# AbnerVictor/OOD-GAN-inversion

Hardware: AMD Instinct MI355X
Metric: 1024² face inversions/sec (100 W+ steps) (higher is better)
Workload: dtype f16-split (hi+lo f16 operands, f32 accumulate): 3 MFMA/product in every forward conv (fp32-equivalent), 2 in the input-gradient convs (back-propagated gradient rounded to f16 before each contraction, weights keep hi+lo); dL/dW+ vs the float64 reference 1.4e-5..3.6e-5 ('f16s': 1.3e-5..2.6e-5, the ref

## Files before the change

### ood-gan-inversion_amd/csrc/common.hpp

```cpp
#pragma once
#include <hip/hip_runtime.h>
#include <cstdio>
#include <cstdarg>
#include <functional>
#include <utility>
#include "../../include/oodgan.h"

namespace oodgan {
struct PlanRec;
extern thread_local PlanRec* tl_plan_rec;
extern int g_null_launch;
void plan_append(std::function<void()>&& f);
template <class F>
inline void launch_rec(F&& f) {
    f();
    if (__builtin_expect(tl_plan_rec != nullptr, 0)) plan_append(std::function<void()>(std::forward<F>(f)));
}
}
#undef hipLaunchKernelGGL
#define hipLaunchKernelGGL(kernelName, numBlocks, numThreads, memPerBlock, streamId, ...)                                        \
    ::oodgan::launch_rec([=]() {                                                                                                 \
        if (!::oodgan::g_null_launch) (kernelName)<<<(numBlocks), (numThreads), (memPerBlock), (streamId)>>>(__VA_ARGS__);      \
    })

namespace oodgan {

void set_error(const char* fmt, ...);

enum { OODGAN_TUN_S1_BIG_MIN_ITEMS = 0, OODGAN_TUN_S2_BIG_MIN_ITEMS, OODGAN_TUN_T2_BIG_MIN_ITEMS, OODGAN_TUN_BLURT_STRIP, OODGAN_TUN_BLUR_STRIP, OODGAN_TUN_UPVB_WAVES, OODGAN_TUN_FEWOUT_QUAD, OODGAN_TUN_TINY_MID_MAX, OODGAN_TUN_STRIPX_WAVES, OODGAN_TUN_COUNT };
long tunable(int id);

enum { OODGAN_DC_STRIPX = 0, OODGAN_DC_STRIP, OODGAN_DC_S1BIG, OODGAN_DC_S1V2, OODGAN_DC_S1PP, OODGAN_DC_TINY, OODGAN_DC_T2BIG,
       OODGAN_DC_T2V2, OODGAN_DC_T2GEN, OODGAN_DC_S2BIG, OODGAN_DC_S2V2, OODGAN_DC_S2GEN, OODGAN_DC_UPVB,
       OODGAN_DC_S1BIG_YS, OODGAN_DC_S2BIG_FUSE, OODGAN_DC_S2BIG_DOTXS,
       OODGAN_DC_S1BIG_G2, OODGAN_DC_S2BIG_G2, OODGAN_DC_STRIPX_G2, OODGAN_DC_S2BIG_XH, OODGAN_DC_S1BIG_XH,
       OODGAN_DC_COMPOSITE_MSE,
       OODGAN_DC_SSIM, OODGAN_DC_COUNT };
void count_dispatch(int id);

bool bound_device_ok(const char* what);

inline int check_launch(const char* what) {
    hipError_t e = hipGetLastError();
    if (e != hipSuccess) {
        set_error("%s: %s", what, hipGetErrorString(e));
        return OODGAN_E_LAUNCH;
    }
    return OODGAN_OK;
}

#define OODGAN_REQUIRE(cond, ...)          \
    do {                                    \
        if (!(cond)) {                      \
            oodgan::set_error(__VA_ARGS__); \
            return OODGAN_E_ARG;            \
        }                                   \
    } while (0)

constexpr float kSqrt2 = 1.4142135623730951f;
constexpr float kInvPos = 1.f / kSqrt2, kInvNeg = 1.f / (0.2f * kSqrt2);
constexpr int kWave = 64;

inline hipStream_t as_stream(void* s) { return reinterpret_cast<hipStream_t>(s); }

inline int stream_grid(long work_items, int block) {
    long g = (work_items + block - 1) / block;
    if (g > 2048) g = 2048;
    if (g < 1) g = 1;
    return static_cast<int>(g);
}

__device__ __forceinline__ float wave_sum(float v) {
#pragma unroll
    for (int o = 32; o > 0; o >>= 1) v += __shfl_xor(v, o, 64);
    return v;
}

__device__ __forceinline__ float row_sum16(const float* __restrict__ p, int n, int l) {
    float v[4];
#pragma unroll
    for (int u = 0; u < 4; ++u) v[u] = p[min(l + 16 * u, n - 1)];
#pragma unroll
    for (int u = 0; u < 4; ++u) v[u] = l + 16 * u < n ? v[u] : 0.f;
    float r = (v[0] + v[1]) + (v[2] + v[3]);
    r += __shfl_xor(r, 8, 64);
    r += __shfl_xor(r, 4, 64);
    r += __shfl_xor(r, 2, 64);
    r += __shfl_xor(r, 1, 64);
    return r;
}

__device__ __forceinline__ float row_sum_wave(const float* __restrict__ p, int n, int lane) {
    float a0 = 0.f, a1 = 0.f, a2 = 0.f, a3 = 0.f;
    for (int i0 = lane; i0 < n; i0 += 512) {
        float v[8];
#pragma unroll
        for (int u = 0; u < 8; ++u) v[u] = p[min(i0 + 64 * u, n - 1)];
#pragma unroll
        for (int u = 0; u < 8; ++u) v[u] = i0 + 64 * u < n ? v[u] : 0.f;
        a0 += v[0] + v[4]; a1 += v[1] + v[5]; a2 += v[2] + v[6]; a3 += v[3] + v[7];
    }
    return wave_sum((a0 + a1) + (a2 + a3));
}

__device__ __forceinline__ float row_sum(const float* __restrict__ p, int n, int lane) {
    return n <= 64 ? row_sum16(p, n, lane & 15) : row_sum_wave(p, n, lane);
}

__device__ __forceinline__ float demod_dot(const float* __restrict__ sp, const float* __restrict__ wp, int Ci, int lane) {
    float a0 = 0.f, a1 = 0.f, a2 = 0.f, a3 = 0.f;
    for (int c0 = lane; c0 < Ci; c0 += 512) {
        float sv[8], wv[8];
#pragma unroll
        for (int u = 0; u < 8; ++u) {
            const int ci = min(c0 + 64 * u, Ci - 1);
            sv[u] = sp[ci];
            wv[u] = wp[ci];
        }
#pragma unroll
        for (int u = 0; u < 8; ++u) {
            const float pr = c0 + 64 * u < Ci ? sv[u] * sv[u] * wv[u] : 0.f;
            if ((u & 3) == 0) a0 += pr; else if ((u & 3) == 1) a1 += pr; else if ((u & 3) == 2) a2 += pr; else a3 += pr;
        }
    }
    return wave_sum((a0 + a1) + (a2 + a3));
}

#ifndef OODGAN_NT_STREAM
#define OODGAN_NT_STREAM 1
#endif
typedef float oodgan_f4v __attribute__((ext_vector_type(4)));
typedef float oodgan_f2v __attribute__((ext_vector_type(2)));
typedef unsigned oodgan_u4v __attribute__((ext_vector_type(4)));
__device__ __forceinline__ float4 ld4_stream(const float* p) {
#if OODGAN_NT_STREAM
    const oodgan_f4v v = __builtin_nontemporal_load(reinterpret_cast<const oodgan_f4v*>(p));
    return make_float4(v.x, v.y, v.z, v.w);
#else
    return *reinterpret_cast<const float4*>(p);
#endif
}
__device__ __forceinline__ float2 ld2_stream(const float* p) {
#if OODGAN_NT_STREAM
    const oodgan_f2v v = __builtin_nontemporal_load(reinterpret_cast<const oodgan_f2v*>(p));
    return make_float2(v.x, v.y);
#else
    return *reinterpret_cast<const float2*>(p);
#endif
}
__device__ __forceinline__ float ld1_stream(const float* p) {
#if OODGAN_NT_STREAM
    return __builtin_nontemporal_load(p);
#else
    return *p;
#endif
}
__device__ __forceinline__ void st4_stream(float* p, float4 v) {
#if OODGAN_NT_STREAM
    __builtin_nontemporal_store(oodgan_f4v{v.x, v.y, v.z, v.w}, reinterpret_cast<oodgan_f4v*>(p));
#else
    *reinterpret_cast<float4*>(p) = v;
#endif
}
template <typename T16>
__device__ __forceinline__ void st16_stream(void* p, const T16& v) {
    static_assert(sizeof(T16) == 16, "16-byte value");
#if OODGAN_NT_STREAM
    __builtin_nontemporal_store(__builtin_bit_cast(oodgan_u4v, v), reinterpret_cast<oodgan_u4v*>(p));
#else
    *reinterpret_cast<T16*>(p) = v;
#endif
}

template <int CTRL, int ROW_MASK>
__device__ __forceinline__ float dpp_take(float v) {
    return __builtin_bit_cast(float, __builtin_amdgcn_update_dpp(0, __builtin_bit_cast(int, v), CTRL, ROW_MASK, 0xF, false));
}
__device__ __forceinline__ float half_sum_dpp(float v) {
    v += dpp_take<0xB1, 0xF>(v);
    v += dpp_take<0x4E, 0xF>(v);
    v += dpp_take<0x141, 0xF>(v);
    v += dpp_take<0x140, 0xF>(v);
    v += dpp_take<0x142, 0xA>(v);
    return v;
}
constexpr int kHalfSumLane = 31;

__device__ __forceinline__ float block_sum_256(float v, float* red ) {
    v = wave_sum(v);
    const int lane = threadIdx.x & 63, wv = threadIdx.x >> 6;
    __syncthreads();
    if (lane == 0) red[wv] = v;
    __syncthreads();
    return red[0] + red[1] + red[2] + red[3];
}

}
```

### ood-gan-inversion_amd/csrc/conv_f16s_s2big.hip

```cpp
#include "conv_common.hpp"
#include "sform.hpp"
#include <cstdint>
#include <cstdlib>
#include <type_traits>

using namespace oodgan;

typedef _Float16 half8 __attribute__((ext_vector_type(8)));
typedef __attribute__((address_space(3))) void lds_void;

#ifdef OODGAN_CLOCK_STAMP
__device__ unsigned long long* g_s2big_stamp = nullptr;
__device__ long g_s2big_stamp_n = 0;
#define S2_STAMP(i) do { if (FUSE && (wave == 0 || wave == 7)) stv[i] = __builtin_amdgcn_s_memtime(); } while (0)
#else
#define S2_STAMP(i)
#endif

namespace {

constexpr int SB_ROWS = 9, SB_C = 33;
constexpr int SB_ROWSLOTS = 2 * SB_C * 4;
constexpr int SB_XSLOTS = SB_ROWS * SB_ROWSLOTS;
constexpr int SB_XPIECES = 40;
constexpr int SB_XBYTES = SB_XPIECES * 1024;

struct SPDims2 { int KC, Hq, Wq; long plane; };

__host__ __device__ inline SPDims2 sp_dims2(int C, int H, int W) {
    SPDims2 d;
    d.KC = (C + 15) / 16;
    d.Hq = (H + 7) / 8 * 8 + 2;
    d.Wq = (W + 31) / 32 * 32 + 2;
    d.plane = (long)d.Hq * d.Wq * 4;
    return d;
}

struct S2Big {
    oodgan_conv_args a;
    const uint4* xs;
    SPDims2 sp;
    const float* w_unscale;
    int Hout, Wout, tiles_x, tiles_y, mblocks, Mp;
    long out_plane;
    int ablate;
    oodgan_actbwd_fuse f;
    SDims yd;
};

template <int MH>
struct S2Cfg {
    static constexpr int RW = MH == 2 ? 2 : 1;
    static constexpr int NRG = 8 / RW;
    static constexpr int MBW = 64 * MH;
    static constexpr int TAPB = 4 * MBW * 16;
    static constexpr int PPT = TAPB / 1024;
    static constexpr int WA = 6 * PPT / 8, WB = (3 * PPT + 7) / 8;
    static constexpr int NA = 5 + WA, NB = 5 + WB;
    static constexpr int OFF_XA = 0, OFF_WA = SB_XBYTES, OFF_XB = OFF_WA + 6 * TAPB, OFF_WB = OFF_XB + SB_XBYTES;
    static constexpr int SMEM = OFF_WB + 3 * TAPB;
    static constexpr int OFF_CST = SMEM;
    static constexpr int SMEM_FUSE = SMEM + 8 * MBW * 4;
};

constexpr int vmcnt_imm(int n) { return ((n >> 4) & 3) << 14 | 0x0F70 | (n & 15); }

typedef _Float16 half2v __attribute__((ext_vector_type(2)));

template <bool DOT, int MH, bool FUSE = false, bool G2 = false>
__global__ __launch_bounds__(512) void conv_f16s_s2big_kernel(const S2Big p, const uint4* __restrict__ wpk16) {
    using C = S2Cfg<MH>;
    constexpr int RW = C::RW;
    extern __shared__ __attribute__((aligned(16))) unsigned char smem[];
    const oodgan_conv_args& a = p.a;
    const int tid = threadIdx.x, lane = tid & 63;
    const int wave = __builtin_amdgcn_readfirstlane(tid >> 6);
    const int l31 = lane & 31, half = lane >> 5;
    const int rg = wave % C::NRG, mh = wave / C::NRG;

#ifdef OODGAN_CLOCK_STAMP
    unsigned long long stv[8] = {0, 0, 0, 0, 0, 0, 0, 0};
#endif
    S2_STAMP(0);
    int w = xcd_remap(blockIdx.x, gridDim.x);
    const int mblk = w % p.mblocks;
    w /= p.mblocks;
    const int ntile = p.tiles_x * p.tiles_y;
    const int tile = w % ntile, b = w / ntile;
    const int ty = tile / p.tiles_x, tx = tile % p.tiles_x;
    const int r0 = ty * 8, c0 = tx * 32, m0 = mblk * C::MBW;
    const int H = p.Hout, W = p.Wout, M = a.M;

    const bool xh = G2 && a.x_hi_only == 2;
    unsigned offx[5];
    bool xok[5];
#pragma unroll
    for (int i = 0; i < 5; ++i) {
        int P = (wave + 8 * i) * 64 + lane;
        if (P >= SB_XSLOTS) P = SB_XSLOTS - 1;
        const int row = P / SB_ROWSLOTS, rem = P % SB_ROWSLOTS;
        const int px = rem / (SB_C * 4), q = rem % (SB_C * 4);
        const int c = q >> 2, s = ((q & 3) - ((c >> 2) & 3)) & 3;
        if (xh) {
            offx[i] = (unsigned)(((long)px * p.sp.plane + ((long)(r0 + row) * p.sp.Wq + (c0 + c)) * 2 + (s & 1)) * 16);
            xok[i] = s < 2;
        } else {
            offx[i] = (unsigned)(((long)px * p.sp.plane + ((long)(r0 + row) * p.sp.Wq + (c0 + c)) * 4 + s) * 16);
            xok[i] = true;
        }
    }
    const long plane_bytes = p.sp.plane * 16;
    const int grp = a.groups > 1 ? m0 / (M / a.groups) : 0;
    const unsigned char* xb = reinterpret_cast<const unsigned char*>(p.xs) + ((long)b * p.sp.KC + (long)grp * ((a.K + 15) / 16)) * 4 * plane_bytes;
    const unsigned char* wb = reinterpret_cast<const unsigned char*>(wpk16) + (long)m0 * 16;
    const unsigned lane16 = lane * 16;
    const long wchunk_bytes = (long)36 * p.Mp * 16;
    const long wrow_bytes = (long)p.Mp * 16;
    const int nchunk = (a.K + 15) / 16;
    const int nstage = 2 * nchunk;

    auto dma_piece = [&](int st, int j) {
        const int t = st >> 1, py = st & 1;
        if (j < 5) {
            unsigned char* dx_ = smem + (py ? C::OFF_XB : C::OFF_XA);
            const unsigned char* xsrc = xb + ((long)t * 4 + py * 2) * plane_bytes;
            if (!G2 || xok[j])
                __builtin_amdgcn_global_load_lds((const __attribute__((address_space(1))) void*)(xsrc + offx[j]),
                                                 (lds_void*)(dx_ + (wave + 8 * j) * 1024), 16, 0, 0);
            return;
        }
        const int i = j - 5;
        const int nw = py ? C::WB : C::WA, npieces = (py ? 3 : 6) * C::PPT;
        if (i >= nw) return;
        unsigned char* dw_ = smem + (py ? C::OFF_WB : C::OFF_WA);
        const unsigned char* wsrc = wb + (long)t * wchunk_bytes;
        int pw = wave + 8 * i;
        if (pw >= npieces) pw -= 8;
        const int sl = pw / C::PPT, q = pw % C::PPT;
        const int tap = py ? 3 + sl : (sl / 3) * 6 + sl % 3;
        const int row = (q * 64) / C::MBW, j0 = (q * 64) % C::MBW;
        const unsigned char* sb = wsrc + (long)(tap * 4 + row) * wrow_bytes + j0 * 16;
        __builtin_amdgcn_global_load_lds((const __attribute__((address_space(1))) void*)(sb + lane16), (lds_void*)(dw_ + pw * 1024), 16, 0, 0);
    };
    auto dma_stage = [&](int st) {
#pragma unroll
        for (int j = 0; j < C::NA; ++j) dma_piece(st, j);
    };

    f32x16 acc[2][RW];
#pragma unroll
    for (int mt = 0; mt < 2; ++mt)
#pragma unroll
        for (int nt = 0; nt < RW; ++nt)
#pragma unroll
            for (int r = 0; r < 16; ++r) acc[mt][nt][r] = 0.f;

    unsigned lrd[2][2];
#pragma unroll
    for (int dxs = 0; dxs < 2; ++dxs)
#pragma unroll
        for (int lo = 0; lo < 2; ++lo) {
            const int c = dxs + l31;
            lrd[dxs][lo] = c * 64 + (((half + 2 * lo + ((c >> 2) & 3)) & 3) << 4);
        }
    const unsigned lwf = (half * C::MBW + mh * 64 + l31) * 16;

    struct Frag { half8 ah[2], al[2], bh[RW], bl[RW]; };
    auto load_tap = [&](Frag& f, const unsigned char* lx, const unsigned char* lw, auto sl_c) {
        constexpr int sl = decltype(sl_c)::value;
        constexpr int arow = sl / 3, kx = sl % 3;
#pragma unroll
        for (int mt = 0; mt < 2; ++mt) {
            f.ah[mt] = *reinterpret_cast<const half8*>(lw + sl * C::TAPB + (0 * 2) * C::MBW * 16 + mt * 32 * 16);
            f.al[mt] = *reinterpret_cast<const half8*>(lw + sl * C::TAPB + (1 * 2) * C::MBW * 16 + mt * 32 * 16);
        }
#pragma unroll
        for (int nt = 0; nt < RW; ++nt) {
            const unsigned char* xr = lx + ((rg * RW + nt + arow) * 2 + (kx & 1)) * (SB_C * 64);
            f.bh[nt] = *reinterpret_cast<const half8*>(xr + lrd[kx >> 1][0]);
            if (!G2) f.bl[nt] = *reinterpret_cast<const half8*>(xr + lrd[kx >> 1][1]);
        }
    };
    auto mfma_tap = [&](const Frag& f) {
#pragma unroll
        for (int mt = 0; mt < 2; ++mt)
#pragma unroll
            for (int nt = 0; nt < RW; ++nt) acc[mt][nt] = __builtin_amdgcn_mfma_f32_32x32x16_f16(f.ah[mt], f.bh[nt], acc[mt][nt], 0, 0, 0);
        if (!G2) {
#pragma unroll
        for (int mt = 0; mt < 2; ++mt)
#pragma unroll
            for (int nt = 0; nt < RW; ++nt) acc[mt][nt] = __builtin_amdgcn_mfma_f32_32x32x16_f16(f.ah[mt], f.bl[nt], acc[mt][nt], 0, 0, 0);
        }
#pragma unroll
        for (int mt = 0; mt < 2; ++mt)
#pragma unroll
            for (int nt = 0; nt < RW; ++nt) acc[mt][nt] = __builtin_amdgcn_mfma_f32_32x32x16_f16(f.al[mt], f.bh[nt], acc[mt][nt], 0, 0, 0);
    };
#define S2B_IC(n) std::integral_constant<int, n>{}
#define S2B_SB() __builtin_amdgcn_sched_barrier(0)

    constexpr bool EARLY = FUSE && MH == 1;
    float eq0 = 0.f, eq1 = 0.f, eq2 = 0.f, enz = 0.f, edv[EARLY ? 2 : 1][16];
    bool eok = false;
    if constexpr (EARLY) {
        static_assert(!EARLY || RW == 1, "one row per wave");
        const oodgan_actbwd_fuse& f = p.f;
        const int px = c0 + l31, py_ = r0 + rg;
        const long HW = (long)H * W, pix = (long)py_ * W + px;
        eok = py_ < H && px < W;
        if (eok) {
            if (f.g_rgb) {
                const float* gr = f.g_rgb + (long)b * 3 * HW + pix;
                eq0 = gr[0]; eq1 = gr[HW]; eq2 = gr[2 * HW];
            }
            if (f.noise) enz = (f.noise_w ? f.noise_w[0] : 1.f) * f.noise[(long)(f.noise_batch > 1 ? b : 0) * HW + pix];
        }
        if (a.dotx_sform) {
#pragma unroll
            for (int mt = 0; mt < 2; ++mt)
#pragma unroll
                for (int blk = 0; blk < 2; ++blk) {
                    const int kc = min((m0 + mh * 64 + mt * 32) / 16 + blk, p.yd.KC - 1);
                    const unsigned char* rec = reinterpret_cast<const unsigned char*>(a.dotx) +
                        sform_unit(p.yd, b, kc, min(py_, H - 1), min(px, W - 1), 0) * 16 + 8 * half;
#pragma unroll
                    for (int sl = 0; sl < 4; ++sl) {
                        const float2 t = *reinterpret_cast<const float2*>(rec + 16 * sl);
                        edv[EARLY ? mt : 0][8 * blk + 2 * sl] = t.x;
                        edv[EARLY ? mt : 0][8 * blk + 2 * sl + 1] = t.y;
                    }
                }
        } else {
#pragma unroll
            for (int mt = 0; mt < 2; ++mt) {
                const float* dr = a.dotx + ((long)b * M + m0 + mh * 64 + mt * 32) * HW + pix;
#pragma unroll
                for (int r = 0; r < 16; ++r) {
                    const int ch = (r & 3) + 8 * (r >> 2) + 4 * half;
                    edv[EARLY ? mt : 0][r] = (eok && m0 + mh * 64 + mt * 32 + ch < M) ? dr[(long)ch * HW] : 0.f;
                }
            }
        }
    }

    float cv[8] = {0.f, 0.f, 0.f, 0.f, 0.f, 0.f, 0.f, 1.f};
    if constexpr (FUSE) {
        const oodgan_actbwd_fuse& f = p.f;
        if (tid < C::MBW) {
            const int m = min(m0 + tid, M - 1);
            cv[0] = a.out_scale ? a.out_scale[(long)b * a.out_scale_stride + m] : 1.f;
            if (f.g_rgb) {
                cv[1] = f.w_rgb[0 * M + m];
                cv[2] = f.w_rgb[1 * M + m];
                cv[3] = f.w_rgb[2 * M + m];
                cv[4] = f.s_rgb[(long)b * f.s_rgb_stride + m];
            }
            if (f.bias) cv[5] = f.bias[m];
            cv[6] = f.dscale[(long)b * f.dscale_stride + m];
            if (a.dotx_sform) {
                const float sc = a.dotx_scale[(long)b * a.dotx_scale_stride + m];
                cv[7] = sc != 0.f ? 1.f / sc : 0.f;
            }
        }
    }
    dma_stage(0);
    if constexpr (FUSE) {
        if (tid < C::MBW) {
            const oodgan_actbwd_fuse& f = p.f;
            float* cst = reinterpret_cast<float*>(smem + C::OFF_CST);
            const bool mok = m0 + tid < M;
            cst[0 * C::MBW + tid] = mok ? cv[0] : 0.f;
            cst[1 * C::MBW + tid] = mok ? cv[1] * f.rgb_scale : 0.f;
            cst[2 * C::MBW + tid] = mok ? cv[2] * f.rgb_scale : 0.f;
            cst[3 * C::MBW + tid] = mok ? cv[3] * f.rgb_scale : 0.f;
            cst[4 * C::MBW + tid] = mok ? cv[4] : 0.f;
            cst[5 * C::MBW + tid] = mok ? cv[5] : 0.f;
            cst[6 * C::MBW + tid] = mok ? cv[6] * f.mul2[1] : 0.f;
            cst[7 * C::MBW + tid] = mok ? cv[7] : 0.f;
            __builtin_amdgcn_s_waitcnt(0xC07F);
        }
    }
    S2_STAMP(1);
    for (int st = 0; st < nstage; ++st) {
        const int py = st & 1;
        __builtin_amdgcn_s_waitcnt(vmcnt_imm(0));
        __builtin_amdgcn_s_barrier();
        const bool pf = st + 1 < nstage && !(p.ablate & 2);
        if (p.ablate & 1) { if (pf) dma_stage(st + 1); continue; }
        const unsigned char* lx = smem + (py ? C::OFF_XB : C::OFF_XA);
        const unsigned char* lw = smem + (py ? C::OFF_WB : C::OFF_WA) + lwf;
        Frag f0, f1;
        if (MH == 2 && pf) dma_stage(st + 1);
#define S2B_DMA(j) if (MH == 1 && pf) dma_piece(st + 1, (j));
        load_tap(f0, lx, lw, S2B_IC(0));
        S2B_SB();
        if (py == 0) {
            load_tap(f1, lx, lw, S2B_IC(1)); S2B_DMA(0) S2B_DMA(1) S2B_SB(); mfma_tap(f0); S2B_SB();
            load_tap(f0, lx, lw, S2B_IC(2)); S2B_DMA(2) S2B_DMA(3) S2B_SB(); mfma_tap(f1); S2B_SB();
            load_tap(f1, lx, lw, S2B_IC(3)); S2B_DMA(4) S2B_SB(); mfma_tap(f0); S2B_SB();
            load_tap(f0, lx, lw, S2B_IC(4)); S2B_DMA(5) S2B_SB(); mfma_tap(f1); S2B_SB();
            load_tap(f1, lx, lw, S2B_IC(5)); S2B_DMA(6) S2B_SB(); mfma_tap(f0); S2B_SB();
            S2B_DMA(7) S2B_SB();
            mfma_tap(f1);
        } else {
            load_tap(f1, lx, lw, S2B_IC(1)); S2B_DMA(0) S2B_DMA(1) S2B_DMA(2) S2B_DMA(3) S2B_SB(); mfma_tap(f0); S2B_SB();
            load_tap(f0, lx, lw, S2B_IC(2)); S2B_DMA(4) S2B_DMA(5) S2B_DMA(6) S2B_DMA(7) S2B_SB(); mfma_tap(f1); S2B_SB();
            S2B_DMA(8) S2B_DMA(9) S2B_DMA(10) S2B_SB();
            mfma_tap(f0);
        }
#undef S2B_DMA
    }
    __builtin_amdgcn_s_barrier();
    S2_STAMP(2);
#undef S2B_IC
#undef S2B_SB

    if constexpr (FUSE) {
        static_assert(DOT, "the fused epilogue includes the dot");
        const oodgan_actbwd_fuse& f = p.f;
        float* red = reinterpret_cast<float*>(smem);
        float* cst = reinterpret_cast<float*>(smem + C::OFF_CST);
        const float us = (p.w_unscale ? p.w_unscale[0] : 1.f) * (a.in_mul2 ? a.in_mul2[0] : 1.f);
        const float rscale = f.mul2[1];
        const int px = c0 + l31;
        const long HW = (long)H * W;
        const float nw = f.noise ? (f.noise_w ? f.noise_w[0] : 1.f) : 0.f;
        float q0[RW], q1[RW], q2[RW], nzv[RW];
        bool okr[RW];
#pragma unroll
        for (int nt = 0; nt < RW; ++nt) {
            const int py_ = r0 + rg * RW + nt;
            okr[nt] = py_ < H && px < W;
            q0[nt] = q1[nt] = q2[nt] = nzv[nt] = 0.f;
            if constexpr (EARLY) {
                okr[nt] = eok; q0[nt] = eq0; q1[nt] = eq1; q2[nt] = eq2; nzv[nt] = enz;
            } else if (okr[nt]) {
                const long pix = (long)py_ * W + px;
                if (f.g_rgb) {
                    const float* gr = f.g_rgb + (long)b * 3 * HW + pix;
                    q0[nt] = gr[0]; q1[nt] = gr[HW]; q2[nt] = gr[2 * HW];
                }
                if (f.noise) nzv[nt] = nw * f.noise[(long)(f.noise_batch > 1 ? b : 0) * HW + pix];
            }
        }
        float vmaxv = 0.f;
#pragma unroll
        for (int mt = 0; mt < 2; ++mt) {
            if (MH == 2) __builtin_amdgcn_sched_barrier(0);
            const int chb = mh * 64 + mt * 32;
            float dv[RW][16];
            if (a.dotx_sform) {
#pragma unroll
                for (int nt = 0; nt < RW; ++nt) {
                    float raw[16];
                    if constexpr (EARLY) {
#pragma unroll
                        for (int i = 0; i < 16; ++i) raw[i] = edv[EARLY ? mt : 0][i];
                    } else {
                        const int py_ = r0 + rg * RW + nt;
#pragma unroll
                        for (int blk = 0; blk < 2; ++blk) {
                            const int kc = min((m0 + chb) / 16 + blk, p.yd.KC - 1);
                            const unsigned char* rec = reinterpret_cast<const unsigned char*>(a.dotx) +
                                sform_unit(p.yd, b, kc, min(py_, H - 1), min(px, W - 1), 0) * 16 + 8 * half;
#pragma unroll
                            for (int sl = 0; sl < 4; ++sl) {
                                const float2 t = *reinterpret_cast<const float2*>(rec + 16 * sl);
                                raw[8 * blk + 2 * sl] = t.x;
                                raw[8 * blk + 2 * sl + 1] = t.y;
                            }
                        }
                    }
#pragma unroll
                    for (int r = 0; r < 16; ++r) {
                        const int blk = r >> 3, sl = (r >> 2) & 1, el = r & 3;
                        const unsigned wh = __float_as_uint(raw[8 * blk + 2 * sl + (el >> 1)]), wl = __float_as_uint(raw[8 * blk + 2 * (2 + sl) + (el >> 1)]);
                        const unsigned short bh = (unsigned short)((el & 1) ? (wh >> 16) : (wh & 0xFFFFu)), bl = (unsigned short)((el & 1) ? (wl >> 16) : (wl & 0xFFFFu));
                        const float v = (float)__builtin_bit_cast(_Float16, bh) + (float)__builtin_bit_cast(_Float16, bl);
                        const float inv = cst[7 * C::MBW + chb + (r & 3) + 8 * (r >> 2) + 4 * half];
                        dv[nt][r] = okr[nt] ? v * inv : 0.f;
                    }
                }
            } else {
            const unsigned char* ub = reinterpret_cast<const unsigned char*>(a.dotx + ((long)b * M + m0 + chb) * HW);
#pragma unroll
            for (int nt = 0; nt < RW; ++nt) {
                const int py_ = r0 + rg * RW + nt;
                const unsigned voff = (unsigned)((((long)min(py_, H - 1) * W + min(px, W - 1)) + (long)(4 * half) * HW) * 4);
#pragma unroll
                for (int r = 0; r < 16; ++r) {
                    if constexpr (EARLY) dv[nt][r] = edv[EARLY ? mt : 0][r];
                    else dv[nt][r] = *reinterpret_cast<const float*>(ub + (long)((r & 3) + 8 * (r >> 2)) * HW * 4 + voff);
                }
                if constexpr (!EARLY) {
#pragma unroll
                    for (int r = 0; r < 16; ++r) dv[nt][r] = okr[nt] ? dv[nt][r] : 0.f;
                }
            }
            }
#ifdef OODGAN_CLOCK_STAMP
            asm volatile("" : "+v"(dv[0][0]), "+v"(dv[0][15]));
            if (mt == 0) S2_STAMP(3);
#endif
            unsigned hi[RW][8], lo[RW][8];
#pragma unroll
            for (int r2 = 0; r2 < 8; ++r2) {
                float vv[RW][2];
                const int ch0 = chb + ((2 * r2) & 3) + 8 * ((2 * r2) >> 2) + 4 * half;
                float2 k7[7];
#pragma unroll
                for (int i = 0; i < 7; ++i) k7[i] = *reinterpret_cast<const float2*>(cst + i * C::MBW + ch0);
#pragma unroll
                for (int e = 0; e < 2; ++e) {
                    const int r = 2 * r2 + e;
                    const int ch = ch0 + e;
                    const float c_g = e ? k7[0].y : k7[0].x, w0 = e ? k7[1].y : k7[1].x, w1 = e ? k7[2].y : k7[2].x, w2 = e ? k7[3].y : k7[3].x;
                    const float srg = e ? k7[4].y : k7[4].x, bv = e ? k7[5].y : k7[5].x, ds = e ? k7[6].y : k7[6].x;
                    float ad = 0.f, ar = 0.f, at = 0.f;
#pragma unroll
                    for (int nt = 0; nt < RW; ++nt) {
                        const float a0 = acc[mt][nt][r] * us;
                        const float o = dv[nt][r];
                        ad += a0 * o;
                        const float t = w0 * q0[nt] + w1 * q1[nt] + w2 * q2[nt];
                        const float g = a0 * c_g + srg * t;
                        const float gp = okr[nt] ? g * (o > 0.f ? kSqrt2 : 0.2f * kSqrt2) : 0.f;
                        const float ycv = (o > 0.f ? o * kInvPos : o * kInvNeg) - nzv[nt] - bv;
                        ar += gp * ycv;
                        at += o * t;
                        const float v = gp * ds;
                        vmaxv = fmaxf(vmaxv, fabsf(v));
                        vv[nt][e] = v;
                    }
                    const float v0 = half_sum_dpp(ad), v1 = half_sum_dpp(ar), v2 = half_sum_dpp(at);
                    if (l31 == kHalfSumLane) {
                        red[(rg * 3 + 0) * C::MBW + ch] = v0;
                        red[(rg * 3 + 1) * C::MBW + ch] = v1;
                        red[(rg * 3 + 2) * C::MBW + ch] = v2;
                    }
                }
                if (f.ys_hi_only) {
#pragma unroll
                    for (int nt = 0; nt < RW; ++nt) {
                        half2v h2;
                        h2[0] = (_Float16)vv[nt][0];
                        h2[1] = (_Float16)vv[nt][1];
                        hi[nt][r2] = __builtin_bit_cast(unsigned, h2);
                        lo[nt][r2] = 0u;
                    }
                } else {
#pragma unroll
                    for (int nt = 0; nt < RW; ++nt) split_pair(vv[nt][0], vv[nt][1], hi[nt][r2], lo[nt][r2]);
                }
            }
#pragma unroll
            for (int nt = 0; nt < RW; ++nt) {
                const int py_ = r0 + rg * RW + nt;
#pragma unroll
                for (int cb = 0; cb < 2; ++cb) {
                    auto h0 = __builtin_amdgcn_permlane32_swap(hi[nt][cb * 4 + 0], hi[nt][cb * 4 + 2], false, false);
                    auto h1 = __builtin_amdgcn_permlane32_swap(hi[nt][cb * 4 + 1], hi[nt][cb * 4 + 3], false, false);
                    const int kc = (m0 + chb) / 16 + cb;
                    if (f.ys_hi_only) {
                        if (okr[nt] && kc < p.yd.KC) {
                            uint4* rec = reinterpret_cast<uint4*>(f.ys) + (((long)b * p.yd.KC + kc) * p.yd.plane + ((long)(py_ + 1) * p.yd.Wp + (px + 1)) * 2);
                            rec[half] = make_uint4(h0[0], h1[0], h0[1], h1[1]);
                        }
                        continue;
                    }
                    auto l0 = __builtin_amdgcn_permlane32_swap(lo[nt][cb * 4 + 0], lo[nt][cb * 4 + 2], false, false);
                    auto l1 = __builtin_amdgcn_permlane32_swap(lo[nt][cb * 4 + 1], lo[nt][cb * 4 + 3], false, false);
                    if (okr[nt] && kc < p.yd.KC) {
                        uint4* rec = reinterpret_cast<uint4*>(f.ys) + sform_unit(p.yd, b, kc, py_, px, 0);
                        rec[half] = make_uint4(h0[0], h1[0], h0[1], h1[1]);
                        rec[2 + half] = make_uint4(l0[0], l1[0], l0[1], l1[1]);
                    }
                }
            }
#ifdef OODGAN_CLOCK_STAMP
            __builtin_amdgcn_sched_barrier(0);
            if (mt == 0) S2_STAMP(4); else S2_STAMP(5);
#endif
        }
#pragma unroll
        for (int o = 32; o > 0; o >>= 1) vmaxv = fmaxf(vmaxv, __shfl_xor(vmaxv, o, 64));
        if (lane == 0) f.part_max[(((long)b * ntile + tile) * p.mblocks + mblk) * 8 + wave] = vmaxv / rscale;
        __syncthreads();
        if (tid < C::MBW && m0 + tid < M) {
            float v0 = 0.f, v1 = 0.f, v2 = 0.f;
#pragma unroll
            for (int g = 0; g < C::NRG; ++g) {
                v0 += red[(g * 3 + 0) * C::MBW + tid];
                v1 += red[(g * 3 + 1) * C::MBW + tid];
                v2 += red[(g * 3 + 2) * C::MBW + tid];
            }
            const long o = ((long)b * M + m0 + tid) * a.dot_nparts + tile;
            a.dot_part[o] = v0;
            f.part_r[o] = v1;
            if (f.part_t) f.part_t[o] = v2;
        }
#ifdef OODGAN_CLOCK_STAMP
        S2_STAMP(6);
        if (lane == 0 && (wave == 0 || wave == 7) && g_s2big_stamp && (long)blockIdx.x < g_s2big_stamp_n) {
            unsigned long long* q = g_s2big_stamp + ((long)blockIdx.x * 2 + (wave ? 1 : 0)) * 8;
#pragma unroll
            for (int i = 0; i < 7; ++i) q[i] = stv[i];
            q[7] = __builtin_amdgcn_s_memrealtime();
        }
#endif
        return;
    }
    const float us = (p.w_unscale ? p.w_unscale[0] : 1.f) * (a.in_mul2 ? a.in_mul2[0] : 1.f);
    const int px = c0 + l31;
    float dsum[2][16];
#pragma unroll
    for (int mt = 0; mt < 2; ++mt)
#pragma unroll
        for (int r = 0; r < 16; ++r) dsum[mt][r] = 0.f;
#pragma unroll
    for (int mt = 0; mt < 2; ++mt) {
        float osc[16], bia[16], slp[16];
        unsigned moff[16], doff[16];
        const float* dmy = reinterpret_cast<const float*>(wpk16);
        const float* oscp = a.out_scale ? a.out_scale + (long)b * a.out_scale_stride : dmy;
        const float* biap = (!DOT && a.bias) ? a.bias : dmy;
        const float* slpp = (!DOT && a.act == OODGAN_ACT_PRELU) ? a.slope : dmy;
        float c_o[16], c_b[16], c_s[16];
#pragma unroll
        for (int r = 0; r < 16; ++r) {
            const int mc = min(m0 + mh * 64 + mt * 32 + (r & 3) + 8 * (r >> 2) + 4 * half, M - 1);
            c_o[r] = oscp[a.out_scale ? mc : 0];
            c_b[r] = biap[(!DOT && a.bias) ? mc : 0];
            c_s[r] = slpp[(!DOT && a.act == OODGAN_ACT_PRELU) ? mc : 0];
        }
#pragma unroll
        for (int r = 0; r < 16; ++r) {
            const int m = m0 + mh * 64 + mt * 32 + (r & 3) + 8 * (r >> 2) + 4 * half;
            const bool mok = m < M;
            osc[r] = mok ? (a.out_scale ? c_o[r] : 1.f) * us : 0.f;
            bia[r] = (!DOT && a.bias && mok) ? c_b[r] : 0.f;
            slp[r] = (!DOT && a.act == OODGAN_ACT_PRELU && mok) ? c_s[r] : 1.f;
            moff[r] = mok ? (unsigned)((long)m * p.out_plane * 4) : 0xFFFFFFFFu;
            doff[r] = mok ? (unsigned)((long)m * H * W * 4) : 0u;
        }
        const bool mfull = m0 + mh * 64 + mt * 32 + 32 <= M;
#pragma unroll
        for (int nt = 0; nt < RW; ++nt) {
            const int py_ = r0 + rg * RW + nt;
            const bool ok = py_ < H && px < W;
            unsigned char* yr = reinterpret_cast<unsigned char*>(a.y) + ((long)b * M * p.out_plane + (long)py_ * a.out_pitch + px) * 4;
            const unsigned char* dr = DOT ? reinterpret_cast<const unsigned char*>(a.dotx) + ((long)b * M * H * W + (long)py_ * W + px) * 4 : nullptr;
            float dv[16];
            if (DOT) {
#pragma unroll
                for (int r = 0; r < 16; ++r) dv[r] = 0.f;
                if (ok) {
                    if (mfull) {
#pragma unroll
                        for (int r = 0; r < 16; ++r) dv[r] = *reinterpret_cast<const float*>(dr + doff[r]);
                    } else {
#pragma unroll
                        for (int r = 0; r < 16; ++r)
                            if (moff[r] != 0xFFFFFFFFu) dv[r] = *reinterpret_cast<const float*>(dr + doff[r]);
                    }
                }
#pragma unroll
                for (int r = 0; r < 16; ++r) dsum[mt][r] += (acc[mt][nt][r] * us) * dv[r];
            }
            if (ok && a.y) {
                float o[16];
#pragma unroll
                for (int r = 0; r < 16; ++r) {
                    o[r] = acc[mt][nt][r] * osc[r];
                    if (!DOT) {
                        o[r] += bia[r];
                        if (a.act == OODGAN_ACT_LRELU) o[r] = (o[r] > 0.f ? o[r] : 0.2f * o[r]) * kSqrt2;
                        else if (a.act == OODGAN_ACT_PRELU) o[r] = o[r] > 0.f ? o[r] : slp[r] * o[r];
                    }
                }
                if (mfull) {
#pragma unroll
                    for (int r = 0; r < 16; ++r) *reinterpret_cast<float*>(yr + moff[r]) = o[r];
                } else {
#pragma unroll
                    for (int r = 0; r < 16; ++r)
                        if (moff[r] != 0xFFFFFFFFu) *reinterpret_cast<float*>(yr + moff[r]) = o[r];
                }
            }
        }
    }
    if (DOT) {
        float* red = reinterpret_cast<float*>(smem);
#pragma unroll
        for (int mt = 0; mt < 2; ++mt)
#pragma unroll
            for (int r = 0; r < 16; ++r) {
                const float v = half_sum_dpp(dsum[mt][r]);
                if (l31 == kHalfSumLane) red[rg * C::MBW + mh * 64 + mt * 32 + (r & 3) + 8 * (r >> 2) + 4 * half] = v;
            }
        __syncthreads();
        if (tid < C::MBW && m0 + tid < M) {
            float v = 0.f;
#pragma unroll
            for (int g = 0; g < C::NRG; ++g) v += red[g * C::MBW + tid];
            a.dot_part[((long)b * M + m0 + tid) * a.dot_nparts + tile] = v;
        }
    }
}

}

namespace oodgan {

bool s2_big_eligible(const oodgan_conv_args& a) {
    if (!(a.mode == OODGAN_CONV_S2 && a.x_sform && a.ys == nullptr && a.in_scale == nullptr && a.in_shift == nullptr &&
          a.noise == nullptr && (a.y != nullptr || a.dotx != nullptr) && a.M >= 64))
        return false;
    if ((a.bias != nullptr || a.act != OODGAN_ACT_NONE) && (a.dotx != nullptr || a.fuse != nullptr || a.y == nullptr)) return false;
    if (a.groups > 1 && (a.dotx != nullptr || a.fuse != nullptr || a.K % 16 != 0 || a.M % a.groups != 0 || (a.M / a.groups) % 128 != 0)) return false;
    if (a.fuse) return true;
    const int Hn = (a.Hin - 1) / 2, Wn = (a.Win - 1) / 2;
    const long items = (long)((Hn + 7) / 8) * ((Wn + 31) / 32) * a.B * ((a.M + 63) / 64);
    return items >= tunable(OODGAN_TUN_S2_BIG_MIN_ITEMS);
}

}

extern "C" int oodgan_conv3x3_s2_fuse_supported(int B, int K, int M, int Hin, int Win) {
    oodgan_conv_args a = {};
    a.mode = OODGAN_CONV_S2; a.x_sform = 1; a.B = B; a.K = K; a.M = M; a.Hin = Hin; a.Win = Win;
    a.y = reinterpret_cast<float*>(1);
    return (M % 32) == 0 && oodgan::s2_big_eligible(a) ? 1 : 0;
}

extern "C" int oodgan_conv3x3_s2_grouped_supported(int B, int K, int M, int groups, int Hin, int Win) {
    oodgan_conv_args a = {};
    a.mode = OODGAN_CONV_S2; a.x_sform = 1; a.B = B; a.K = K; a.M = M; a.Hin = Hin; a.Win = Win; a.groups = groups;
    a.y = reinterpret_cast<float*>(1);
    return groups > 1 && oodgan::s2_big_eligible(a) ? 1 : 0;
}

#ifdef OODGAN_CLOCK_STAMP
extern "C" int oodgan_debug_set_s2big_stamp_buffer(void* buf, long n) {
    unsigned long long* q = reinterpret_cast<unsigned long long*>(buf);
    if (hipMemcpyToSymbol(HIP_SYMBOL(g_s2big_stamp), &q, sizeof(q)) != hipSuccess ||
        hipMemcpyToSymbol(HIP_SYMBOL(g_s2big_stamp_n), &n, sizeof(n)) != hipSuccess) {
        oodgan::set_error("debug_set_s2big_stamp_buffer: hipMemcpyToSymbol failed");
        return OODGAN_E_LAUNCH;
    }
    return 0;
}
#endif

namespace oodgan {

int launch_s2_big(const oodgan_conv_args& a_in, const void* wpk16, const float* unscale, hipStream_t st) {
    S2Big p;
    p.a = a_in;
    oodgan_conv_args& a = p.a;
    p.Hout = (a.Hin - 1) / 2;
    p.Wout = (a.Win - 1) / 2;
    if (a.out_pitch == 0) a.out_pitch = p.Wout;
    p.out_plane = (long)p.Hout * a.out_pitch;
    p.xs = reinterpret_cast<const uint4*>(a.x);
    p.sp = sp_dims2(a.K * (a.groups > 1 ? a.groups : 1), p.Hout, p.Wout);
    p.w_unscale = unscale;
    p.tiles_y = (p.Hout + 7) / 8;
    p.tiles_x = (p.Wout + 31) / 32;
    p.Mp = (a.M + 63) / 64 * 64;
    const long items128 = (long)p.tiles_x * p.tiles_y * a.B * (a.M / 128);
    const bool mh2 = (a.M % 128) == 0 && items128 >= 256;
    p.mblocks = mh2 ? a.M / 128 : (a.M + 63) / 64;
    if (a.dotx) {
        OODGAN_REQUIRE(a.dot_part != nullptr, "conv3x3: dotx without dot_part");
        OODGAN_REQUIRE(a.dot_nparts == p.tiles_x * p.tiles_y, "conv3x3 f16s S2: dot_nparts %d != %d", a.dot_nparts, p.tiles_x * p.tiles_y);
    }
    OODGAN_REQUIRE((long)a.M * p.out_plane * 4 < (1L << 32), "conv3x3 S2 big: plane too large");
    const bool fuse = a.fuse != nullptr;
    p.yd = sform_dims(a.M, p.Hout, p.Wout);
    if (fuse) {
        p.f = *a.fuse;
        OODGAN_REQUIRE(a.dotx && a.dot_part && p.f.ys && p.f.part_r && p.f.part_max && p.f.dscale && p.f.mul2 && (a.M % 32) == 0,
                       "conv3x3 S2 fused activation backward: needs dotx, ys, part_r, part_max, dscale, mul2 and M %% 32 == 0");
        OODGAN_REQUIRE(!p.f.g_rgb || (p.f.w_rgb && p.f.s_rgb && p.f.part_t), "conv3x3 S2 fused: rgb branch needs w_rgb, s_rgb and part_t");
        OODGAN_REQUIRE(p.f.noise == nullptr || p.f.noise_batch == 1 || p.f.noise_batch == a.B, "conv3x3 S2 fused: noise_batch");
        OODGAN_REQUIRE(p.f.nmax >= (long)a.B * p.tiles_x * p.tiles_y * p.mblocks * 8, "conv3x3 S2 fused: part_max too small");
    }
    OODGAN_REQUIRE(p.sp.plane * 32 < (1L << 32), "conv3x3 S2 big: input plane too large");
#ifdef OODGAN_DEBUG_ABLATE
    static const int abl = getenv("OODGAN_S2BIG_ABLATE") ? atoi(getenv("OODGAN_S2BIG_ABLATE")) : 0;
    p.ablate = abl;
#else
    p.ablate = 0;
#endif
    const long total = (long)p.tiles_x * p.tiles_y * a.B * p.mblocks;
    OODGAN_REQUIRE(total > 0 && total < (1L << 31), "conv3x3: grid too large");
    static bool once = ((void)hipFuncSetAttribute(reinterpret_cast<const void*>(&conv_f16s_s2big_kernel<true, 2>), hipFuncAttributeMaxDynamicSharedMemorySize, S2Cfg<2>::SMEM),
                        (void)hipFuncSetAttribute(reinterpret_cast<const void*>(&conv_f16s_s2big_kernel<false, 2>), hipFuncAttributeMaxDynamicSharedMemorySize, S2Cfg<2>::SMEM),
                        (void)hipFuncSetAttribute(reinterpret_cast<const void*>(&conv_f16s_s2big_kernel<true, 1>), hipFuncAttributeMaxDynamicSharedMemorySize, S2Cfg<1>::SMEM),
                        (void)hipFuncSetAttribute(reinterpret_cast<const void*>(&conv_f16s_s2big_kernel<false, 1>), hipFuncAttributeMaxDynamicSharedMemorySize, S2Cfg<1>::SMEM),
                        (void)hipFuncSetAttribute(reinterpret_cast<const void*>(&conv_f16s_s2big_kernel<true, 2, true>), hipFuncAttributeMaxDynamicSharedMemorySize, S2Cfg<2>::SMEM_FUSE),
                        (void)hipFuncSetAttribute(reinterpret_cast<const void*>(&conv_f16s_s2big_kernel<true, 1, true>), hipFuncAttributeMaxDynamicSharedMemorySize, S2Cfg<1>::SMEM_FUSE),
                        (void)hipFuncSetAttribute(reinterpret_cast<const void*>(&conv_f16s_s2big_kernel<true, 2, false, true>), hipFuncAttributeMaxDynamicSharedMemorySize, S2Cfg<2>::SMEM),
                        (void)hipFuncSetAttribute(reinterpret_cast<const void*>(&conv_f16s_s2big_kernel<true, 1, false, true>), hipFuncAttributeMaxDynamicSharedMemorySize, S2Cfg<1>::SMEM),
                        (void)hipFuncSetAttribute(reinterpret_cast<const void*>(&conv_f16s_s2big_kernel<true, 2, true, true>), hipFuncAttributeMaxDynamicSharedMemorySize, S2Cfg<2>::SMEM_FUSE),
                        (void)hipFuncSetAttribute(reinterpret_cast<const void*>(&conv_f16s_s2big_kernel<true, 1, true, true>), hipFuncAttributeMaxDynamicSharedMemorySize, S2Cfg<1>::SMEM_FUSE), true);
    (void)once;
    const uint4* w16 = reinterpret_cast<const uint4*>(wpk16);
    const bool g2 = a.x_hi_only != 0 && a.dotx != nullptr;
    OODGAN_REQUIRE(a.x_hi_only != 2 || (g2 && a.groups <= 1), "conv3x3 S2 big: hi-only input records (x_hi_only = 2) need dotx (the two-instruction instances) and no groups");
    if (g2) {
        count_dispatch(OODGAN_DC_S2BIG_G2);
        if (a.x_hi_only == 2) count_dispatch(OODGAN_DC_S2BIG_XH);
        if (fuse) {
            if (mh2) hipLaunchKernelGGL((conv_f16s_s2big_kernel<true, 2, true, true>), dim3((unsigned)total), dim3(512), S2Cfg<2>::SMEM_FUSE, st, p, w16);
            else hipLaunchKernelGGL((conv_f16s_s2big_kernel<true, 1, true, true>), dim3((unsigned)total), dim3(512), S2Cfg<1>::SMEM_FUSE, st, p, w16);
        } else if (mh2) hipLaunchKernelGGL((conv_f16s_s2big_kernel<true, 2, false, true>), dim3((unsigned)total), dim3(512), S2Cfg<2>::SMEM, st, p, w16);
        else hipLaunchKernelGGL((conv_f16s_s2big_kernel<true, 1, false, true>), dim3((unsigned)total), dim3(512), S2Cfg<1>::SMEM, st, p, w16);
    } else if (fuse) {
        if (mh2) hipLaunchKernelGGL((conv_f16s_s2big_kernel<true, 2, true>), dim3((unsigned)total), dim3(512), S2Cfg<2>::SMEM_FUSE, st, p, w16);
        else hipLaunchKernelGGL((conv_f16s_s2big_kernel<true, 1, true>), dim3((unsigned)total), dim3(512), S2Cfg<1>::SMEM_FUSE, st, p, w16);
    } else if (mh2) {
        if (a.dotx) hipLaunchKernelGGL((conv_f16s_s2big_kernel<true, 2>), dim3((unsigned)total), dim3(512), S2Cfg<2>::SMEM, st, p, w16);
        else hipLaunchKernelGGL((conv_f16s_s2big_kernel<false, 2>), dim3((unsigned)total), dim3(512), S2Cfg<2>::SMEM, st, p, w16);
    } else {
        if (a.dotx) hipLaunchKernelGGL((conv_f16s_s2big_kernel<true, 1>), dim3((unsigned)total), dim3(512), S2Cfg<1>::SMEM, st, p, w16);
        else hipLaunchKernelGGL((conv_f16s_s2big_kernel<false, 1>), dim3((unsigned)total), dim3(512), S2Cfg<1>::SMEM, st, p, w16);
    }
    return check_launch("conv3x3_f16s_s2big");
}

}
```

Before: 7.804.

## Batch half-wave reductions with permlane16/DPP butterfly and hoist edge masking

Replaces the per-channel 32-lane DPP reduction in the stride-2 fused backward conv epilogue with a transposing butterfly (HalfReduce16). It reduces 16 channels at once via permlane16_swap and DPP merges, so each lane ends up owning a distinct channel's sum, and the results are written with fewer LDS stores. It also moves the weight unscale multiply out of the inner loop into per-channel constants and the final dot write. Out-of-range masking is applied only on edge tiles, once up front, instead of per element. The intent is to cut cross-lane instruction count and per-element selects in the epilogue, at the cost of more intricate lane-index bookkeeping.

```diff
diff --git a/ood-gan-inversion_amd/csrc/common.hpp b/ood-gan-inversion_amd/csrc/common.hpp
--- a/ood-gan-inversion_amd/csrc/common.hpp
+++ b/ood-gan-inversion_amd/csrc/common.hpp
@@ -186,6 +186,29 @@
 }
 constexpr int kHalfSumLane = 31;
 
+template <int CTRL, int BANK_MASK>
+__device__ __forceinline__ float dpp_merge(float old, float v) {
+    return __builtin_bit_cast(float, __builtin_amdgcn_update_dpp(__builtin_bit_cast(int, old), __builtin_bit_cast(int, v), CTRL, 0xF, BANK_MASK, false));
+}
+__device__ __forceinline__ int half_reduce16_index(int lane) { return ((lane >> 4) & 1) | ((lane >> 2) & 2) | (lane & 4); }
+struct HalfReduce16 {
+    float lv[3], out[2];
+    __device__ __forceinline__ void push(int r, float v) {
+        if ((r & 1) == 0) { lv[0] = v; return; }
+        const auto sw = __builtin_amdgcn_permlane16_swap(__builtin_bit_cast(unsigned, lv[0]), __builtin_bit_cast(unsigned, v), false, false);
+        unsigned s0 = sw[0], s1 = sw[1];
+        asm("" : "+v"(s0), "+v"(s1));
+        v = __builtin_bit_cast(float, s0) + __builtin_bit_cast(float, s1);
+        if ((r & 2) == 0) { lv[1] = v; return; }
+        v = dpp_merge<0x140, 0xC>(lv[1], v) + dpp_merge<0x140, 0x3>(v, lv[1]);
+        if ((r & 4) == 0) { lv[2] = v; return; }
+        v = dpp_merge<0x141, 0xA>(lv[2], v) + dpp_merge<0x141, 0x5>(v, lv[2]);
+        v += dpp_take<0xB1, 0xF>(v);
+        v += dpp_take<0x4E, 0xF>(v);
+        out[r >> 3] = v;
+    }
+};
+
 __device__ __forceinline__ float block_sum_256(float v, float* red ) {
     v = wave_sum(v);
     const int lane = threadIdx.x & 63, wv = threadIdx.x >> 6;
diff --git a/ood-gan-inversion_amd/csrc/conv_f16s_s2big.hip b/ood-gan-inversion_amd/csrc/conv_f16s_s2big.hip
--- a/ood-gan-inversion_amd/csrc/conv_f16s_s2big.hip
+++ b/ood-gan-inversion_amd/csrc/conv_f16s_s2big.hip
@@ -245,6 +245,7 @@
     }
 
     float cv[8] = {0.f, 0.f, 0.f, 0.f, 0.f, 0.f, 0.f, 1.f};
+    const float us_f = FUSE ? (p.w_unscale ? p.w_unscale[0] : 1.f) * (a.in_mul2 ? a.in_mul2[0] : 1.f) : 1.f;
     if constexpr (FUSE) {
         const oodgan_actbwd_fuse& f = p.f;
         if (tid < C::MBW) {
@@ -270,7 +271,7 @@
             const oodgan_actbwd_fuse& f = p.f;
             float* cst = reinterpret_cast<float*>(smem + C::OFF_CST);
             const bool mok = m0 + tid < M;
-            cst[0 * C::MBW + tid] = mok ? cv[0] : 0.f;
+            cst[0 * C::MBW + tid] = mok ? cv[0] * us_f : 0.f;
             cst[1 * C::MBW + tid] = mok ? cv[1] * f.rgb_scale : 0.f;
             cst[2 * C::MBW + tid] = mok ? cv[2] * f.rgb_scale : 0.f;
             cst[3 * C::MBW + tid] = mok ? cv[3] * f.rgb_scale : 0.f;
@@ -321,7 +322,6 @@
         const oodgan_actbwd_fuse& f = p.f;
         float* red = reinterpret_cast<float*>(smem);
         float* cst = reinterpret_cast<float*>(smem + C::OFF_CST);
-        const float us = (p.w_unscale ? p.w_unscale[0] : 1.f) * (a.in_mul2 ? a.in_mul2[0] : 1.f);
         const float rscale = f.mul2[1];
         const int px = c0 + l31;
         const long HW = (long)H * W;
@@ -344,6 +344,22 @@
                 if (f.noise) nzv[nt] = nw * f.noise[(long)(f.noise_batch > 1 ? b : 0) * HW + pix];
             }
         }
+        const bool edge = r0 + 8 > H || c0 + 32 > W;
+        if (edge) {
+#pragma unroll
+            for (int mt = 0; mt < 2; ++mt)
+#pragma unroll
+                for (int nt = 0; nt < RW; ++nt)
+#pragma unroll
+                    for (int r = 0; r < 16; ++r) {
+                        acc[mt][nt][r] = okr[nt] ? acc[mt][nt][r] : 0.f;
+                        if constexpr (EARLY) edv[EARLY ? mt : 0][r] = eok ? edv[EARLY ? mt : 0][r] : 0.f;
+                    }
+        }
+        float k_sp = kSqrt2, k_sn = 0.2f * kSqrt2, k_ip = kInvPos, k_in = kInvNeg;
+        asm volatile("" : "+v"(k_sp), "+v"(k_sn), "+v"(k_ip), "+v"(k_in));
+        const int own = half_reduce16_index(lane);
+        const int own_ch = (own & 3) + 8 * (own >> 2) + 4 * half;
         float vmaxv = 0.f;
 #pragma unroll
         for (int mt = 0; mt < 2; ++mt) {
@@ -371,6 +387,10 @@
                                 raw[8 * blk + 2 * sl + 1] = t.y;
                             }
                         }
+                        if (edge) {
+#pragma unroll
+                            for (int i = 0; i < 16; ++i) raw[i] = okr[nt] ? raw[i] : 0.f;
+                        }
                     }
 #pragma unroll
                     for (int r = 0; r < 16; ++r) {
@@ -379,7 +399,7 @@
                         const unsigned short bh = (unsigned short)((el & 1) ? (wh >> 16) : (wh & 0xFFFFu)), bl = (unsigned short)((el & 1) ? (wl >> 16) : (wl & 0xFFFFu));
                         const float v = (float)__builtin_bit_cast(_Float16, bh) + (float)__builtin_bit_cast(_Float16, bl);
                         const float inv = cst[7 * C::MBW + chb + (r & 3) + 8 * (r >> 2) + 4 * half];
-                        dv[nt][r] = okr[nt] ? v * inv : 0.f;
+                        dv[nt][r] = v * inv;
                     }
                 }
             } else {
@@ -394,8 +414,10 @@
                     else dv[nt][r] = *reinterpret_cast<const float*>(ub + (long)((r & 3) + 8 * (r >> 2)) * HW * 4 + voff);
                 }
                 if constexpr (!EARLY) {
-#pragma unroll
-                    for (int r = 0; r < 16; ++r) dv[nt][r] = okr[nt] ? dv[nt][r] : 0.f;
+                    if (edge) {
+#pragma unroll
+                        for (int r = 0; r < 16; ++r) dv[nt][r] = okr[nt] ? dv[nt][r] : 0.f;
+                    }
                 }
             }
             }
@@ -404,6 +426,7 @@
             if (mt == 0) S2_STAMP(3);
 #endif
             unsigned hi[RW][8], lo[RW][8];
+            HalfReduce16 sum_d, sum_r, sum_t;
 #pragma unroll
             for (int r2 = 0; r2 < 8; ++r2) {
                 float vv[RW][2];
@@ -420,25 +443,23 @@
                     float ad = 0.f, ar = 0.f, at = 0.f;
 #pragma unroll
                     for (int nt = 0; nt < RW; ++nt) {
-                        const float a0 = acc[mt][nt][r] * us;
+                        const float a0 = acc[mt][nt][r];
                         const float o = dv[nt][r];
                         ad += a0 * o;
                         const float t = w0 * q0[nt] + w1 * q1[nt] + w2 * q2[nt];
                         const float g = a0 * c_g + srg * t;
-                        const float gp = okr[nt] ? g * (o > 0.f ? kSqrt2 : 0.2f * kSqrt2) : 0.f;
-                        const float ycv = (o > 0.f ? o * kInvPos : o * kInvNeg) - nzv[nt] - bv;
+                        const bool pos = o > 0.f;
+                        const float gp = g * (pos ? k_sp : k_sn);
+                        const float ycv = o * (pos ? k_ip : k_in) - nzv[nt] - bv;
                         ar += gp * ycv;
                         at += o * t;
                         const float v = gp * ds;
                         vmaxv = fmaxf(vmaxv, fabsf(v));
                         vv[nt][e] = v;
                     }
-                    const float v0 = half_sum_dpp(ad), v1 = half_sum_dpp(ar), v2 = half_sum_dpp(at);
-                    if (l31 == kHalfSumLane) {
-                        red[(rg * 3 + 0) * C::MBW + ch] = v0;
-                        red[(rg * 3 + 1) * C::MBW + ch] = v1;
-                        red[(rg * 3 + 2) * C::MBW + ch] = v2;
-                    }
+                    sum_d.push(r, ad);
+                    sum_r.push(r, ar);
+                    sum_t.push(r, at);
                 }
                 if (f.ys_hi_only) {
 #pragma unroll
@@ -452,6 +473,14 @@
                 } else {
 #pragma unroll
                     for (int nt = 0; nt < RW; ++nt) split_pair(vv[nt][0], vv[nt][1], hi[nt][r2], lo[nt][r2]);
+                }
+            }
+            if ((lane & 3) == 0) {
+#pragma unroll
+                for (int m = 0; m < 2; ++m) {
+                    red[(rg * 3 + 0) * C::MBW + chb + own_ch + 16 * m] = sum_d.out[m];
+                    red[(rg * 3 + 1) * C::MBW + chb + own_ch + 16 * m] = sum_r.out[m];
+                    red[(rg * 3 + 2) * C::MBW + chb + own_ch + 16 * m] = sum_t.out[m];
                 }
             }
 #pragma unroll
@@ -496,7 +525,7 @@
                 v2 += red[(g * 3 + 2) * C::MBW + tid];
             }
             const long o = ((long)b * M + m0 + tid) * a.dot_nparts + tile;
-            a.dot_part[o] = v0;
+            a.dot_part[o] = v0 * us_f;
             f.part_r[o] = v1;
             if (f.part_t) f.part_t[o] = v2;
         }
@@ -593,12 +622,16 @@
     if (DOT) {
         float* red = reinterpret_cast<float*>(smem);
 #pragma unroll
-        for (int mt = 0; mt < 2; ++mt)
-#pragma unroll
-            for (int r = 0; r < 16; ++r) {
-                const float v = half_sum_dpp(dsum[mt][r]);
-                if (l31 == kHalfSumLane) red[rg * C::MBW + mh * 64 + mt * 32 + (r & 3) + 8 * (r >> 2) + 4 * half] = v;
-            }
+        for (int mt = 0; mt < 2; ++mt) {
+            HalfReduce16 hs;
+#pragma unroll
+            for (int r = 0; r < 16; ++r) hs.push(r, dsum[mt][r]);
+            const int own = half_reduce16_index(lane);
+            if ((lane & 3) == 0) {
+#pragma unroll
+                for (int m = 0; m < 2; ++m) red[rg * C::MBW + mh * 64 + mt * 32 + (own & 3) + 8 * (own >> 2) + 4 * half + 16 * m] = hs.out[m];
+            }
+        }
         __syncthreads();
         if (tid < C::MBW && m0 + tid < M) {
             float v = 0.f;
```

After: 7.855 (median of 5 runs). No clear change (+0.7%).
